# ChaoqinRobotics/LINS---LiDAR-inertial-SLAM

Hardware: NVIDIA H100
Metric: ESKF iterations/sec (higher is better)
Workload: dtype f64 (f32 association)

## Files before the change

lins---lidar-inertial-slam_b200/csrc/cuda/lins_assoc.cuh:

```cuda
#pragma once
#include "lins_assoc_az.cuh"

namespace lins_dev {

#ifndef LINS_SEARCH_DIAG
#define LINS_SEARCH_DIAG 0
#endif
constexpr bool kSearchDiag = LINS_SEARCH_DIAG != 0;
#ifndef LINS_GROUP_LANES
#define LINS_GROUP_LANES 4
#endif
constexpr int kGroupLanes = LINS_GROUP_LANES;
#ifndef LINS_THREAD_SCAN_BINS
#define LINS_THREAD_SCAN_BINS 16
#endif
#ifndef LINS_THREAD_WALK_BINS
#define LINS_THREAD_WALK_BINS 48
#endif
constexpr int kThreadScanBins = LINS_THREAD_SCAN_BINS, kThreadWalkBins = LINS_THREAD_WALK_BINS;

struct PassBuffers {
  float4* qpt;
  float4* sel;
  unsigned long long* key;
  int* pos;
  float4* qa;
  int4* qw;
  float4* qref;
  float4* qref2;
  int* qccr;
  float4* qext;
  int* wl;
  double* wacc;
  int* wcnt;
  int nvw;
};

struct PassLayout {
  size_t slots;
  size_t fixed_bytes;
  size_t query_bytes;
};

__host__ __device__ constexpr size_t align16(size_t b) { return (b + 15) & ~(size_t)15; }

__host__ __device__ __forceinline__ PassLayout pass_layout(int nslots, int qtile, PassBuffers* pb = nullptr, unsigned char* smem = nullptr,
                                                           unsigned char* qscratch = nullptr, unsigned cta = 0, size_t qscratch_stride = 0) {
  static_assert(sizeof(Smem) % 16 == 0, "slots are indexed as an array");
  const int NQ = nslots * qtile;
  const size_t nvw_all = (size_t)nslots * (qtile / 32);
  const size_t wacc_bytes = align16(nvw_all * kNAcc * sizeof(double)), wcnt_bytes = align16(nvw_all * 2 * sizeof(int));
  PassLayout lay;
  lay.slots = align16(sizeof(CtaMem));
  lay.fixed_bytes = lay.slots + nslots * sizeof(Smem) + wacc_bytes + wcnt_bytes;
  lay.query_bytes = align16((size_t)NQ * (sizeof(*pb->qpt) + sizeof(*pb->sel) + sizeof(*pb->qa) + sizeof(*pb->qw) + sizeof(*pb->qref) +
                                          sizeof(*pb->qref2) + sizeof(*pb->qext) + sizeof(*pb->key) + 3 * sizeof(*pb->pos) +
                                          sizeof(*pb->qccr) + sizeof(*pb->wl)));
  if (pb) {
    PassBuffers& b = *pb;
    b.nvw = qtile / 32;
    unsigned char* p = smem + lay.slots;
    p += nslots * sizeof(Smem);
    b.wacc = reinterpret_cast<double*>(p); p += wacc_bytes;
    b.wcnt = reinterpret_cast<int*>(p); p += wcnt_bytes;
    if (qscratch) p = qscratch + (size_t)cta * qscratch_stride;
    b.qpt = reinterpret_cast<float4*>(p); p = reinterpret_cast<unsigned char*>(b.qpt + NQ);
    b.sel = reinterpret_cast<float4*>(p); p = reinterpret_cast<unsigned char*>(b.sel + NQ);
    b.qa = reinterpret_cast<float4*>(p); p = reinterpret_cast<unsigned char*>(b.qa + NQ);
    b.qw = reinterpret_cast<int4*>(p); p = reinterpret_cast<unsigned char*>(b.qw + NQ);
    b.qref = reinterpret_cast<float4*>(p); p = reinterpret_cast<unsigned char*>(b.qref + NQ);
    b.qref2 = reinterpret_cast<float4*>(p); p = reinterpret_cast<unsigned char*>(b.qref2 + NQ);
    b.qext = reinterpret_cast<float4*>(p); p = reinterpret_cast<unsigned char*>(b.qext + NQ);
    b.key = reinterpret_cast<unsigned long long*>(p); p = reinterpret_cast<unsigned char*>(b.key + NQ);
    b.pos = reinterpret_cast<int*>(p); p = reinterpret_cast<unsigned char*>(b.pos + 3 * NQ);
    b.qccr = reinterpret_cast<int*>(p); p = reinterpret_cast<unsigned char*>(b.qccr + NQ);
    b.wl = reinterpret_cast<int*>(p);
  }
  return lay;
}

__device__ __forceinline__ AzIndex az_index_of(const Smem& sm, const BatchView& bv, bool surf) {
  AzIndex ix;
  if (surf) { ix.pts = bv.az_s + sm.ts0; ix.bstart = sm.azTabS; ix.elev = sm.elevS; ix.nb = sm.nbS; ix.nrings = sm.nringsS; ix.T = sm.Ts; }
  else { ix.pts = bv.az_c + sm.tc0; ix.bstart = sm.azTabC; ix.elev = sm.elevC; ix.nb = sm.nbC; ix.nrings = sm.nringsC; ix.T = sm.Tc; }
  return ix;
}

__device__ __forceinline__ int slot_of(int v, int Q) { return (v >= Q) + (v >= 2 * Q) + (v >= 3 * Q); }

template <int MODE>
__device__ void association_pass(CtaMem& cta, Smem* slots, const BatchView& bv, const KParams& kp, const PassBuffers& pb) {
  const int Q = bv.qtile, NQ = bv.nslots * Q;
  const float nearf = (float)kp.nearest_sq;
  const int warp = threadIdx.x >> 5, lane = threadIdx.x & 31;
  const int toff = cta.pass_first ? 32 : 0;

  for (int v = threadIdx.x; v < NQ; v += kThreads) {
    const int sl = slot_of(v, Q), i = v - sl * Q;
    Smem& sm = slots[sl];
    if (!sm.run || i >= sm.ns + sm.nc) continue;
    const float4 s = transform_to_start(pb.qpt[v], sm, kp.scan_period);
    pb.sel[v] = s;
    pb.key[v] = kKeyMax;
    const bool search = (sm.iter % kp.icp_freq) == 0;
    if (!search) {
      if (!sm.pos_valid) {
        if (i < sm.ns) { const int* o = bv.ind_s + 3 * (size_t)(sm.qs0 + i); pb.pos[3 * v] = o[0]; pb.pos[3 * v + 1] = o[1]; pb.pos[3 * v + 2] = o[2]; }
        else { const int* o = bv.ind_c + 2 * (size_t)(sm.qc0 + i - sm.ns); pb.pos[3 * v] = o[0]; pb.pos[3 * v + 1] = o[1]; pb.pos[3 * v + 2] = -1; }
      }
      continue;
    }
    if (!sm.az_ok) continue;
    const bool surf = i < sm.ns;
    const bool seeded = !sm.first_pass;
    const AzIndex ixq = az_index_of(sm, bv, surf);
    float4 qa = make_float4(0.f, 0.f, -1.f, 0.f);
    if (seeded) {
      const float4 r1 = pb.qref[v], r2 = pb.qref2[v], ex = pb.qext[v];
      const unsigned nearbits = __float_as_uint(nearf);
      const int w1s = pb.pos[3 * v], w2s = pb.pos[3 * v + 1], w3s = pb.pos[3 * v + 2];
      const int r1s = __float_as_int(ex.y), r2s = __float_as_int(ex.z), r3s = __float_as_int(ex.w);
      const int ccr0 = pb.qccr[v];
      const bool walks = ccr0 >= 0;
      auto entry = [&](int slot, bool use) -> float4 {
        return use && slot >= 0 && slot < ixq.T ? ixq.pts[slot] : make_float4(0.f, 0.f, 0.f, 0.f);
      };
      const float4 tw1 = entry(w1s, true), tr1 = entry(r1s, w1s >= 0);
      const float4 tw2 = entry(w2s, walks), tr2 = entry(r2s, walks && w2s >= 0);
      const float4 tw3 = entry(w3s, walks && surf), tr3 = entry(r3s, walks && surf && w3s >= 0);
      const float moved1 = sqrtf(sqdist_f32(s.x, s.y, s.z, r1.x, r1.y, r1.z));
      const bool ok1 = w1s >= 0 ? cert_accepted<false>(tw1, tr1, s, r1s, r1.w, moved1, nearbits, 0) : cert_rejected(r1.w, moved1);
      bool ok2 = false;
      if (ok1 && walks) {
        const int c0 = ccr0 & 0x00ffffff;
        const float moved2 = sqrtf(sqdist_f32(s.x, s.y, s.z, r2.x, r2.y, r2.z));
        ok2 = w2s >= 0 ? cert_accepted<true>(tw2, tr2, s, r2s, r2.w, moved2, nearbits, c0) : cert_rejected(r2.w, moved2);
        if (ok2 && surf) ok2 = w3s >= 0 ? cert_accepted<true>(tw3, tr3, s, r3s, ex.x, moved2, nearbits, c0) : cert_rejected(ex.x, moved2);
      }
      if (ok1 && (ok2 || ccr0 < 0)) { pb.qw[v] = make_int4(-2, 0, 0, 0); continue; }
      if (ok1) { az_polar(s, qa); pb.qa[v] = qa; pb.qw[v] = make_int4(-3, 0, 0, 0); continue; }
    }
    const int w1 = az_prepare_nn(ixq, s, nearf, seeded ? pb.pos[3 * v] : -1, (int)pb.qpt[v].w, qa);
    pb.qa[v] = qa;
    pb.qw[v] = make_int4(w1, 0, 0, 0);
    if (sm.first_pass && w1 >= 0 && (w1 & 0xffff) <= kThreadScanBins) pb.wl[NQ - 1 - atomicAdd(&cta.wl_tn[0], 1)] = v;
    else pb.wl[atomicAdd(&cta.wl_n[0], 1)] = v;
    if (bv.timers && w1 >= 0) atomicAdd(&cta.dbg[0], w1 & 0xffff);
  }
  __syncthreads();
  LINS_TICK(3 + toff);

  if (cta.any_indexed) {
    if (bv.timers && threadIdx.x == 0) {
      atomicAdd((unsigned long long*)&bv.timers[10], (unsigned long long)cta.wl_n[0]);
      atomicAdd((unsigned long long*)&bv.timers[12], (unsigned long long)cta.dbg[0]);
    }
    const float gate = sqrtf(nearf);
    auto nn_finish = [&](int v, const AzIndex& ix, const float4 s, const Top3& top, int w1, float Bout) {
      const unsigned long long k1 = top.k1;
      const int p1 = top.p1;
      const float d1 = __uint_as_float((unsigned)(k1 >> 32));
      const bool acc1 = k1 != kKeyMax && p1 >= 0 && (double)d1 < kp.nearest_sq;
      const float bound1 = w1 < 0 ? -1.f : acc1 ? cert_bound(top.d3, Bout) : rejected_slack((unsigned)(k1 >> 32), Bout, gate);
      pb.qref[v] = make_float4(s.x, s.y, s.z, bound1);
      pb.qext[v].y = __int_as_float(acc1 ? top.p2 : -1);
      pb.pos[3 * v] = acc1 ? p1 : -1;
      pb.qccr[v] = acc1 ? ((slot_ring(ix.pts[p1].w) << 24) | (int)(unsigned)(k1 & 0xffffffffu)) : -1;
    };
    constexpr int G = kGroupLanes;
    const int sub = lane & (G - 1), glead = lane & ~(G - 1);
    const unsigned gmask = G == 32 ? 0xffffffffu : (((1u << G) - 1u) << glead);
    for (;;) {
      int k = 0;
      if (sub == 0) k = atomicAdd(&cta.wl_thead[0], 1);
      k = __shfl_sync(gmask, k, glead);
      if (k >= cta.wl_tn[0]) break;
      const int v = pb.wl[NQ - 1 - k];
      const int sl = slot_of(v, Q), i = v - sl * Q;
      const Smem& sm = slots[sl];
      const AzIndex ix = az_index_of(sm, bv, i < sm.ns);
      const float4 s = pb.sel[v];
      const int w1 = pb.qw[v].x;
      const float4 qag = pb.qa[v];
      const Top3 top = az_scan_nn_group<G>(ix, s, w1, qag.y, qag.w, sub, gmask);
      if (sub == 0) nn_finish(v, ix, s, top, w1, qag.w);
    }
    for (;;) {
      int k = 0;
      if (lane == 0) k = atomicAdd(&cta.wl_head[0], 1);
      k = __shfl_sync(0xffffffffu, k, 0);
      if (k >= cta.wl_n[0]) break;
      const int v = pb.wl[k];
      const int sl = slot_of(v, Q), i = v - sl * Q;
      const Smem& sm = slots[sl];
      int w1 = pb.qw[v].x;
      Top3 top;
      top.init();
      const bool surf = i < sm.ns;
      const AzIndex ix = az_index_of(sm, bv, surf);
      const float4 s = pb.sel[v];
      float4 qa = pb.qa[v];
      if (w1 >= 0) {
        const int wp = sm.first_pass ? az_probe_window(ix, qa, w1) : -1;
        if (wp >= 0) {
          const Top3 pr = az_scan_nn(ix, s, wp, qa.y, sqrtf(widen(kProbeSq)));
          if (pr.p1 >= 0) {
            w1 = az_nn_window(ix, az_seed_bound(ix, s, pr.p1, nearf), qa);
            if (lane == 0) pb.qa[v] = qa;
          }
        }
        top = az_scan_nn(ix, s, w1, qa.y, qa.w);
      }
      if (lane == 0) nn_finish(v, ix, s, top, w1, qa.w);
    }
    __syncthreads();
    LINS_TICK(4 + toff);
    for (int v = threadIdx.x; v < NQ; v += kThreads) {
      const int sl = slot_of(v, Q), i = v - sl * Q;
      const Smem& sm = slots[sl];
      if (!sm.run || !sm.az_ok || i >= sm.ns + sm.nc || (sm.iter % kp.icp_freq) != 0) continue;
      const int lvl = pb.qw[v].x;
      if (lvl == -2) continue;
      const bool surf = i < sm.ns;
      const int ccr = pb.qccr[v];
      if (ccr < 0) {
        pb.pos[3 * v + 1] = -1; pb.pos[3 * v + 2] = -1;
        pb.qw[v] = make_int4(-1, 0, 0, 0);
        if (surf) { int* o = bv.ind_s + 3 * (size_t)(sm.qs0 + i); o[0] = -1; o[1] = -1; o[2] = -1; }
        else { int* o = bv.ind_c + 2 * (size_t)(sm.qc0 + i - sm.ns); o[0] = -1; o[1] = -1; }
        continue;
      }
      int w2 = 0, w3 = 0;
      float B2 = 0.f, B3 = 0.f;
      const bool seeded = !sm.first_pass;
      const int sd2 = seeded ? pb.pos[3 * v + 1] : -1, sd3 = seeded ? pb.pos[3 * v + 2] : -1;
      const int c = ccr & 0x00ffffff, cr = (int)((unsigned)ccr >> 24);
      const AzIndex ix = az_index_of(sm, bv, surf);
      const int p1 = pb.pos[3 * v];
      if (surf) az_prepare_walk<true>(ix, pb.sel[v], pb.qa[v], p1, c, cr, sd2, sd3, min(sm.ns, sm.Ts), nearf, w2, w3, B2, B3);
      else az_prepare_walk<false>(ix, pb.sel[v], pb.qa[v], p1, c, cr, sd2, sd3, min(sm.nc, sm.Tc), nearf, w2, w3, B2, B3);
      pb.qw[v] = make_int4(1, w2, w3, ccr);
      reinterpret_cast<float2*>(pb.key)[v] = make_float2(B2, B3);
      if (sm.first_pass && (w2 & 0xffff) <= kThreadWalkBins && (w3 & 0xffff) <= kThreadWalkBins) pb.wl[NQ - 1 - atomicAdd(&cta.wl_tn[1], 1)] = v;
      else pb.wl[atomicAdd(&cta.wl_n[1], 1)] = v;
      if (bv.timers) atomicAdd(&cta.dbg[1], (w2 & 0xffff) + 4 * (w3 & 0xffff));
    }
    __syncthreads();
    if (bv.timers && threadIdx.x == 0) {
      atomicAdd((unsigned long long*)&bv.timers[11], (unsigned long long)cta.wl_n[1]);
      atomicAdd((unsigned long long*)&bv.timers[13], (unsigned long long)cta.dbg[1]);
    }
    auto walk_finish = [&](int v, const Smem& sm, int i, bool surf, const float4 s, int ccr, const WalkOut& wo) {
      pb.pos[3 * v + 1] = wo.pos2; pb.pos[3 * v + 2] = wo.pos3;
      pb.qref2[v] = make_float4(s.x, s.y, s.z, wo.bound2);
      float4 ex = pb.qext[v];
      ex.x = wo.bound3; ex.z = __int_as_float(wo.run2); ex.w = __int_as_float(wo.run3);
      pb.qext[v] = ex;
      const int i1 = ccr & 0x00ffffff;
      if (surf) { int* o = bv.ind_s + 3 * (size_t)(sm.qs0 + i); o[0] = i1; o[1] = wo.i2; o[2] = wo.i3; }
      else { int* o = bv.ind_c + 2 * (size_t)(sm.qc0 + i - sm.ns); o[0] = i1; o[1] = wo.i2; }
    };
    for (;;) {
      int k = 0;
      if (sub == 0) k = atomicAdd(&cta.wl_thead[1], 1);
      k = __shfl_sync(gmask, k, glead);
      if (k >= cta.wl_tn[1]) break;
      const int v = pb.wl[NQ - 1 - k];
      const int sl = slot_of(v, Q), i = v - sl * Q;
      const Smem& sm = slots[sl];
      const int4 w = pb.qw[v];
      const bool surf = i < sm.ns;
      const float2 B = reinterpret_cast<const float2*>(pb.key)[v];
      const float4 s = pb.sel[v];
      const AzIndex ix = az_index_of(sm, bv, surf);
      const WalkOut wo = surf ? az_scan_walk_group<true, G>(ix, s, w.w, w.y, w.z, min(sm.ns, sm.Ts), nearf, B.x, B.y, sub, gmask)
                              : az_scan_walk_group<false, G>(ix, s, w.w, w.y, w.z, min(sm.nc, sm.Tc), nearf, B.x, B.y, sub, gmask);
      if (sub == 0) walk_finish(v, sm, i, surf, s, w.w, wo);
    }
    for (;;) {
      int k = 0;
      if (lane == 0) k = atomicAdd(&cta.wl_head[1], 1);
      k = __shfl_sync(0xffffffffu, k, 0);
      if (k >= cta.wl_n[1]) break;
      const int v = pb.wl[k];
      const int sl = slot_of(v, Q), i = v - sl * Q;
      const Smem& sm = slots[sl];
      const int4 w = pb.qw[v];
      const bool surf = i < sm.ns;
      const float2 B = reinterpret_cast<const float2*>(pb.key)[v];
      const int w2 = w.y, w3 = w.z;
      const float4 s = pb.sel[v];
      const AzIndex ix = az_index_of(sm, bv, surf);
      const WalkOut wo = surf ? az_scan_walk<true>(ix, s, w.w, w2, w3, min(sm.ns, sm.Ts), nearf, B.x, B.y)
                              : az_scan_walk<false>(ix, s, w.w, w2, w3, min(sm.nc, sm.Tc), nearf, B.x, B.y);
      if (lane == 0) walk_finish(v, sm, i, surf, s, w.w, wo);
    }
  }
  if (cta.any_legacy) {
    for (int sl = 0; sl < bv.nslots; ++sl) {
      const Smem& sm = slots[sl];
      if (!sm.run || sm.az_ok || (sm.iter % kp.icp_freq) != 0) continue;
      const bool sep = nn_separate(bv, sm.scan);
      const float4* __restrict__ nnS = sep ? bv.nn_s + bv.nn_s_off[sm.scan] : bv.ts + sm.ts0;
      const float4* __restrict__ nnC = sep ? bv.nn_c + bv.nn_c_off[sm.scan] : bv.tc + sm.tc0;
      const int TnS = sep ? bv.nn_s_off[sm.scan + 1] - bv.nn_s_off[sm.scan] : sm.Ts;
      const int TnC = sep ? bv.nn_c_off[sm.scan + 1] - bv.nn_c_off[sm.scan] : sm.Tc;
      if (sm.ns > 0 && TnS > 0) nn_brute(pb.sel + sl * Q, pb.key + sl * Q, sm.ns, nnS, TnS);
      if (sm.nc > 0 && TnC > 0) nn_brute(pb.sel + sl * Q + sm.ns, pb.key + sl * Q + sm.ns, sm.nc, nnC, TnC);
    }
    __syncthreads();
    for (int sl = 0; sl < bv.nslots; ++sl) {
      const Smem& sm = slots[sl];
      if (!sm.run || sm.az_ok || (sm.iter % kp.icp_freq) != 0) continue;
      const float4* __restrict__ tgtS = bv.ts + sm.ts0;
      const float4* __restrict__ tgtC = bv.tc + sm.tc0;
      const int fwdS = min(sm.ns, sm.Ts), fwdC = min(sm.nc, sm.Tc);
      for (int i = threadIdx.x; i < sm.ns + sm.nc; i += kThreads) {
        const int v = sl * Q + i;
        const bool surf = i < sm.ns;
        const unsigned long long k1 = pb.key[v];
        const float d1 = __uint_as_float((unsigned)(k1 >> 32));
        const int c = (int)(unsigned)(k1 & 0xffffffffu);
        const bool found = (k1 != kKeyMax) && ((double)d1 < kp.nearest_sq) && c < (surf ? sm.Ts : sm.Tc);
        int i1 = -1, i2 = -1, i3 = -1;
        if (found) {
          i1 = c;
          const float4 s = pb.sel[v];
          if (surf) walk_seq<true>(s, c, tgtS, sm.Ts, fwdS, nearf, i2, i3);
          else walk_seq<false>(s, c, tgtC, sm.Tc, fwdC, nearf, i2, i3);
        }
        pb.pos[3 * v] = i1; pb.pos[3 * v + 1] = i2; pb.pos[3 * v + 2] = i3;
        if (surf) { int* o = bv.ind_s + 3 * (size_t)(sm.qs0 + i); o[0] = i1; o[1] = i2; o[2] = i3; }
        else { int* o = bv.ind_c + 2 * (size_t)(sm.qc0 + i - sm.ns); o[0] = i1; o[1] = i2; }
      }
    }
  }
  __syncthreads();
  LINS_TICK(5 + toff);
  if (threadIdx.x == kThreads - 1) { cta.wl_n[0] = 0; cta.wl_n[1] = 0; cta.wl_tn[0] = 0; cta.wl_tn[1] = 0; cta.wl_head[0] = 0; cta.wl_head[1] = 0; cta.wl_thead[0] = 0; cta.wl_thead[1] = 0; cta.dbg[0] = 0; cta.dbg[1] = 0; }

  double* const fold_stage = cta.u.fold[warp];
  for (int v0 = warp * 32; v0 < NQ; v0 += kThreads) {
    const int sl = slot_of(v0, Q), i0 = v0 - sl * Q;
    const Smem& sm = slots[sl];
    const int ntot = sm.ns + sm.nc;
    if (!sm.run || i0 >= ntot) continue;
    const int v = v0 + lane, i = i0 + lane;
    const bool valid = i < ntot;
    const bool surf = i < sm.ns;
    const bool search = (sm.iter % kp.icp_freq) == 0;
    const bool weighted = sm.iter >= kp.icp_freq;
    const bool by_slot = search ? (sm.az_ok != 0) : (sm.pos_valid && sm.pos_is_slot);
    float4 coeff = make_float4(0.f, 0.f, 0.f, 0.f);
    float4 s = make_float4(0.f, 0.f, 0.f, 0.f);
    bool ok = false;
    if (valid) {
      const int i1 = pb.pos[3 * v], i2 = pb.pos[3 * v + 1], i3 = pb.pos[3 * v + 2];
      s = pb.sel[v];
      if (surf) {
        if (i2 >= 0 && i3 >= 0 && i1 >= 0 && i1 < sm.Ts && i2 < sm.Ts && i3 < sm.Ts) {
          const float4* t = by_slot ? bv.az_s + sm.ts0 : bv.ts + sm.ts0;
          ok = plane_residual(s, t[i1], t[i2], t[i3], weighted, coeff);
        }
      } else {
        if (i2 >= 0 && i1 >= 0 && i1 < sm.Tc && i2 < sm.Tc) {
          const float4* t = by_slot ? bv.az_c + sm.tc0 : bv.tc + sm.tc0;
          ok = line_residual(s, t[i1], t[i2], weighted, coeff);
        }
      }
    }
    double g[6] = {0.0, 0.0, 0.0, 0.0, 0.0, 0.0}, r = 0.0;
    if (ok) {
      if (MODE == MODE_ICP_REDUCE) jacobian_row_icp(pb.qpt[v], coeff, sm.phi, kp.scan_period, g, r);
      else jacobian_row(pb.qpt[v], coeff, sm.R, kp.lidar_scale, g, r);
    }
    const int vw = sl * pb.nvw + (i0 >> 5);
    warp_fold_mma(g, r, fold_stage, pb.wacc + vw * kNAcc);
    const unsigned mS = __ballot_sync(0xffffffffu, ok && surf), mC = __ballot_sync(0xffffffffu, ok && !surf);
    if (lane == kNAcc) pb.wcnt[vw * 2] = __popc(mS);
    else if (lane == kNAcc + 1) pb.wcnt[vw * 2 + 1] = __popc(mC);
    if (MODE == MODE_ASSOC && valid) {
      if (surf) {
        const size_t o = (size_t)(sm.qs0 + i);
        if (bv.sel_s) { bv.sel_s[3 * o] = s.x; bv.sel_s[3 * o + 1] = s.y; bv.sel_s[3 * o + 2] = s.z; }
        if (bv.coeff_s) { bv.coeff_s[4 * o] = coeff.x; bv.coeff_s[4 * o + 1] = coeff.y; bv.coeff_s[4 * o + 2] = coeff.z; bv.coeff_s[4 * o + 3] = coeff.w; }
        if (bv.mask_s) bv.mask_s[o] = ok ? 1 : 0;
      } else {
        const size_t o = (size_t)(sm.qc0 + i - sm.ns);
        if (bv.sel_c) { bv.sel_c[3 * o] = s.x; bv.sel_c[3 * o + 1] = s.y; bv.sel_c[3 * o + 2] = s.z; }
        if (bv.coeff_c) { bv.coeff_c[4 * o] = coeff.x; bv.coeff_c[4 * o + 1] = coeff.y; bv.coeff_c[4 * o + 2] = coeff.z; bv.coeff_c[4 * o + 3] = coeff.w; }
        if (bv.mask_c) bv.mask_c[o] = ok ? 1 : 0;
      }
    }
  }
  __syncthreads();
  LINS_TICK(6 + toff);
}

}
```

lins---lidar-inertial-slam_b200/csrc/cuda/lins_assoc_az.cuh:

```cuda
#pragma once
#include "lins_kernels.cuh"

namespace lins_dev {

struct AzIndex {
  const float4* pts;
  const aztab_t* bstart;
  const int (*elev)[2];
  int nb, nrings, T;
};
__device__ __forceinline__ int float_key(float f) { const int i = __float_as_int(f); return i >= 0 ? i : i ^ 0x7fffffff; }
__device__ __forceinline__ float key_float(int k) { return __int_as_float(k >= 0 ? k : k ^ 0x7fffffff); }
__device__ __forceinline__ float slope_of(float x, float y, float z) {
  return __fdiv_rn(z, sqrtf(__fadd_rn(__fmul_rn(x, x), __fmul_rn(y, y))));
}
__device__ __forceinline__ float ring_lower_bound(const AzIndex& ix, int r, float zq, float rq) {
  const float lo = key_float(ix.elev[r][0]), hi = key_float(ix.elev[r][1]);
  const float a = __fmaf_rn(lo, rq, -zq), b = __fmaf_rn(-hi, rq, zq);
  const float m = a > b ? lo : hi;
  const float bound = fmaxf(a, b) * rsqrtf(__fmaf_rn(m, m, 1.f)) * 0.998f - 1.0e-4f;
  return hi - lo < 1.0e30f ? bound : -1.f;
}

__device__ __forceinline__ int az_bin(float x, float y, int nb) {
// ... 307 lines not shown
  }
  {
    const int bq = az_bin_of_angle(qa.x, ix.nb);
    float& U = SURF ? U3 : U2;
    float4 t[8];
    bool ok[8];
#pragma unroll
    for (int k = 0; k < 4; ++k) {
      const int r = cr + (k < 2 ? k - 2 : k - 1);
      const bool rok = r >= 0 && r < ix.nrings;
      const int slot = rok ? (int)ix.bstart[r * ix.nb + bq] : -1;
      t[2 * k] = fetch(slot, ok[2 * k]);
      t[2 * k + 1] = fetch(rok ? slot - 1 : -1, ok[2 * k + 1]);
    }
#pragma unroll
    for (int k = 0; k < 8; ++k) U = seed_bound<SURF, !SURF>(t[k], ok[k], s, c, cr, fwdBound, U);
  }
  int blo, nbins;
  const float Uw2 = widen(U2);
  az_window(ix.nb, qa.x, az_halfwidth(Uw2, qa.y), blo, nbins);
  w2 = pack_window(blo, nbins);
  B2 = nbins >= ix.nb ? 3.0e38f : sqrtf(Uw2);
  if (SURF) {
    const float Uw3 = widen(U3);
    az_window(ix.nb, qa.x, az_halfwidth(Uw3, qa.y), blo, nbins);
    w3 = pack_window(blo, nbins);
    B3 = nbins >= ix.nb ? 3.0e38f : sqrtf(Uw3);
  } else { w3 = w2; B3 = B2; }
}

#ifndef LINS_WALK_IN_FLIGHT
#define LINS_WALK_IN_FLIGHT 4
#endif
constexpr int kWalkInFlight = LINS_WALK_IN_FLIGHT;
#ifndef LINS_GROUP_WALK_IN_FLIGHT
#define LINS_GROUP_WALK_IN_FLIGHT 4
#endif
constexpr int kGroupWalkInFlight = LINS_GROUP_WALK_IN_FLIGHT;
struct WalkOut {
  int i2, i3, pos2, pos3, run2, run3;
  float bound2, bound3;
};
template <bool SURF>
__device__ __forceinline__ WalkOut az_scan_walk(const AzIndex& ix, const float4 s, int ccr, int w2, int w3, int fwdBound, float nearf,
                                                float B2, float B3) {
  const int lane = threadIdx.x & 31;
  const int c = ccr & 0x00ffffff, cr = (int)((unsigned)ccr >> 24);
  Top3 top;
  top.init();
  constexpr int LPR = SURF ? 7 : 8;
  const int q = lane / LPR;
  const bool own = SURF && q >= 4;
  const int r = own ? cr : cr + (q < 2 ? q - 2 : q - 1);
  const int sub = own ? lane - 4 * LPR : lane - q * LPR, step = own ? 4 : LPR;
  const bool cls2 = SURF ? own : true;
  if (r >= 0 && r < ix.nrings) {
    const int win = cls2 ? w2 : w3;
    const int blo = win >> 16, nbins = win & 0xffff, base = r * ix.nb;
    for (int seg = 0; seg < 2; ++seg) {
      int p, pe;
      if (seg == 0) { p = ix.bstart[base + blo]; pe = ix.bstart[base + min(blo + nbins, ix.nb)]; }
      else { const int e1 = blo + nbins - ix.nb; if (e1 <= 0) break; p = ix.bstart[base]; pe = ix.bstart[base + e1]; }
      for (p += sub; p < pe; p += kWalkInFlight * step) {
        float4 tt[kWalkInFlight];
#pragma unroll
        for (int u = 0; u < kWalkInFlight; ++u) tt[u] = ld_slot(ix, p + step * u < pe ? p + step * u : p);
#pragma unroll
        for (int u = 0; u < kWalkInFlight; ++u) {
          const int pu = p + step * u;
          const float4 t = tt[u];
          const unsigned d = __float_as_uint(sqdist_f32(t.x, t.y, t.z, s.x, s.y, s.z));
          const int j = slot_index(t.w);
          const bool fwd = j > c;
          const bool adm = pu < pe && j != c && (!fwd || j < fwdBound);
          const unsigned long long k = adm ? (((unsigned long long)d << 32) | (fwd ? order_fwd(j) : order_bwd(j))) : kKeyMax;
          top.insert(k, pu);
        }
      }
    }
  }
  const float gate = sqrtf(nearf);
  const unsigned nearbits = __float_as_uint(nearf);
  const bool mine2 = cls2;
  Top3 neutral;
  neutral.init();
  WalkOut o;
  auto finish = [&](Top3 t, float Bout, int& idx, int& pos, int& run, float& bound) {
    warp_top3(t);
    const bool ok = (unsigned)(t.k1 >> 32) < nearbits && t.p1 >= 0;
    idx = ok ? order_decode((unsigned)(t.k1 & 0xffffffffu)) : -1;
    pos = ok ? t.p1 : -1;
    run = ok ? t.p2 : -1;
    bound = ok ? cert_bound(t.d3, Bout) : rejected_slack((unsigned)(t.k1 >> 32), Bout, gate);
  };
  finish(mine2 ? top : neutral, B2, o.i2, o.pos2, o.run2, o.bound2);
  if (SURF) finish(mine2 ? neutral : top, B3, o.i3, o.pos3, o.run3, o.bound3);
  else { o.i3 = -1; o.pos3 = -1; o.run3 = -1; o.bound3 = 0.f; }
  return o;
}

template <bool SURF, int G>
__device__ __forceinline__ WalkOut az_scan_walk_group(const AzIndex& ix, const float4 s, int ccr, int w2, int w3, int fwdBound, float nearf,
                                                      float B2, float B3, int sub, unsigned gmask) {
  const int c = ccr & 0x00ffffff, cr = (int)((unsigned)ccr >> 24);
  Top3 t2, t3;
  t2.init(); t3.init();
  auto scan_ring = [&](int r, int win, Top3& top, int start, int step) {
    const int blo = win >> 16, nbins = win & 0xffff, base = r * ix.nb;
    for (int seg = 0; seg < 2; ++seg) {
      int p, pe;
      if (seg == 0) { p = ix.bstart[base + blo]; pe = ix.bstart[base + min(blo + nbins, ix.nb)]; }
      else { const int e1 = blo + nbins - ix.nb; if (e1 <= 0) break; p = ix.bstart[base]; pe = ix.bstart[base + e1]; }
      for (p += start; p < pe; p += kGroupWalkInFlight * step) {
        float4 tt[kGroupWalkInFlight];
#pragma unroll
        for (int u = 0; u < kGroupWalkInFlight; ++u) tt[u] = ld_slot(ix, p + u * step < pe ? p + u * step : p);
#pragma unroll
        for (int u = 0; u < kGroupWalkInFlight; ++u) {
          const int pu = p + u * step;
          const float4 t = tt[u];
          const unsigned d = __float_as_uint(sqdist_f32(t.x, t.y, t.z, s.x, s.y, s.z));
          const int j = slot_index(t.w);
          const bool fwd = j > c;
          const bool adm = pu < pe && j != c && (!fwd || j < fwdBound);
          top.insert(adm ? (((unsigned long long)d << 32) | (fwd ? order_fwd(j) : order_bwd(j))) : kKeyMax, pu);
        }
      }
    }
  };
  if (SURF && cr < ix.nrings) scan_ring(cr, w2, t2, sub, G);
  for (int idx = sub; idx < 4; idx += G) {
    const int r = cr + (idx < 2 ? idx - 2 : idx - 1);
    if (r < 0 || r >= ix.nrings) continue;
    if (SURF) scan_ring(r, w3, t3, 0, 1); else scan_ring(r, w2, t2, 0, 1);
  }
  group_top3<G>(t2, gmask);
  if (SURF) group_top3<G>(t3, gmask);
  const float gate = sqrtf(nearf);
  const unsigned nearbits = __float_as_uint(nearf);
  WalkOut o;
  auto finish = [&](const Top3& t, float Bout, int& idx, int& pos, int& run, float& bound) {
    const bool ok = (unsigned)(t.k1 >> 32) < nearbits && t.p1 >= 0;
    idx = ok ? order_decode((unsigned)(t.k1 & 0xffffffffu)) : -1;
    pos = ok ? t.p1 : -1;
    run = ok ? t.p2 : -1;
    bound = ok ? cert_bound(t.d3, Bout) : rejected_slack((unsigned)(t.k1 >> 32), Bout, gate);
  };
  finish(t2, B2, o.i2, o.pos2, o.run2, o.bound2);
  if (SURF) finish(t3, B3, o.i3, o.pos3, o.run3, o.bound3);
  else { o.i3 = -1; o.pos3 = -1; o.run3 = -1; o.bound3 = 0.f; }
  return o;
}

template <bool WALK>
__device__ __forceinline__ bool cert_accepted(const float4 tw, const float4 tr, const float4 s, int r, float bound, float moved, unsigned nearbits,
                                              int c) {
  auto key_of = [&](const float4 t) -> unsigned long long {
    const unsigned d = __float_as_uint(sqdist_f32(t.x, t.y, t.z, s.x, s.y, s.z));
    const int j = slot_index(t.w);
    const unsigned lo = WALK ? (j > c ? order_fwd(j) : order_bwd(j)) : (unsigned)j;
    return ((unsigned long long)d << 32) | lo;
  };
  const unsigned long long kw = key_of(tw);
  const unsigned dw = (unsigned)(kw >> 32);
  if (!(dw < nearbits)) return false;
  if (r >= 0 && !(kw < key_of(tr))) return false;
  return sqrtf(__uint_as_float(dw)) + moved + 2.0e-4f < bound;
}
__device__ __forceinline__ bool cert_rejected(float slack, float moved) { return slack > 0.f && 2.0f * moved + 2.0e-4f < slack; }

}
```

lins---lidar-inertial-slam_b200/csrc/cuda/lins_kernels.cuh:

```cuda
#pragma once
#include "../../../include/lins_gpu.h"
#include "lins_device_math.cuh"

namespace lins_dev {

#ifndef LINS_THREADS
#define LINS_THREADS 512
#endif
#ifndef LINS_MIN_CTAS
#define LINS_MIN_CTAS 1
#endif
constexpr int kThreads = LINS_THREADS;
constexpr int kMinCtas = LINS_MIN_CTAS;
constexpr int kWarps = kThreads / 32;
constexpr int kMaxSlots = 4;
constexpr int kMaxRing = 128;
constexpr int kNAcc = 28;
constexpr int kNNChunk = 1024;
constexpr int kAzTabS = 4096;
constexpr int kAzTabC = 1024;
constexpr float kPiF = 3.14159265358979f;
constexpr unsigned long long kKeyMax = 0xFFFFFFFFFFFFFFFFull;

enum KernelMode { MODE_IESKF = 0, MODE_ASSOC = 1, MODE_ICP_REDUCE = 2, MODE_JACOBIAN = 3 };

struct BatchView {
  int n_scans;
  const float4* qs; const int* qs_off;
  const float4* qc; const int* qc_off;
  const float4* ts; const int* ts_off;
  const float4* tc; const int* tc_off;
  const float4* nn_s; const int* nn_s_off;
  const float4* nn_c; const int* nn_c_off;
  const unsigned char* nn_stale;
  const double* state_in;
  const double* cov_in;
  double* state_out;
  double* cov_out;
  lins_scan_result* results;
  lins_report* reports;
  int* ind_s;
  int* ind_c;
  float* sel_s; float* sel_c;
  float* coeff_s; float* coeff_c;
  unsigned char* mask_s; unsigned char* mask_c;
  double* accum;
  float4* az_s; float4* az_c;
  int* work_counter;
  long long* timers;
  int qtile;
  int nslots;
  const int* icp_done;
  unsigned char* qscratch;
  size_t qscratch_stride;
};

struct IcpState {
  double matP[36];
  int iters, converged, done, pad;
};
constexpr int kIcpDoneStride = (int)(sizeof(IcpState) / sizeof(int));
static_assert(sizeof(IcpState) % sizeof(int) == 0, "IcpState stride");

struct KParams {
  int num_iter, icp_freq, force_all_iters, mode, iter0;
  double nearest_sq, lidar_std, lidar_scale, scan_period;
};

__device__ __forceinline__ bool nn_separate(const BatchView& bv, int scan) {
  return bv.nn_s != nullptr && (bv.nn_stale == nullptr || bv.nn_stale[scan] != 0);
}

__device__ __forceinline__ unsigned long long pack_key(float d, unsigned int lo) {
  return ((unsigned long long)__float_as_uint(d) << 32) | lo;
}
__device__ __forceinline__ unsigned long long shfl_xor_u64(unsigned long long v, int m) {
  return __shfl_xor_sync(0xffffffffu, v, m);
}
__device__ __forceinline__ unsigned long long warp_min_u64(unsigned long long v) {
#pragma unroll
  for (int m = 16; m > 0; m >>= 1) {
    unsigned long long o = shfl_xor_u64(v, m);
    v = o < v ? o : v;
  }
  return v;
}

typedef unsigned short aztab_t;

struct alignas(16) Smem {
  double prior[20];
  double Pc[18 * 6];
  double lin[20];
  double phi[3];
  double R[9];
  double Rinv[9];
  double dvec[18];
  double acc[kNAcc + 4];
  double A6[36];
  double y6[6];
  double M6[36];
  double X6[6];
  double upd[18];
  double residualNorm;
  int flags[4];
  int cnt[2];
  int scan;
  int iter;
  int fresh;
  int run;
  int finished;
  int first_pass;
  int pos_valid, pos_is_slot;
  int qs0, ns, qc0, nc, ts0, Ts, tc0, Tc;
  int sortedS, sortedC;
  int az_ok;
  int nbS, nbC, nringsS, nringsC;
  aztab_t azTabS[kAzTabS + 2];
  aztab_t azTabC[kAzTabC + 2];
  int elevS[kMaxRing][2], elevC[kMaxRing][2];
};

struct CtaMem {
  union {
    unsigned build_tab[kAzTabS / 2 + 1];
    struct { double P[324], X[324], U[108], V[108], X6[72]; } ex;
    double fold[kWarps][64];
  } u;
  int scan_tmp[kThreads];
  int wl_n[2], wl_head[2];
  int wl_tn[2], wl_thead[2];
  int dbg[2];
  int n_active, any_fresh, any_finished, any_legacy, any_indexed, exhausted, pass_first;
  unsigned long long mbar;
  unsigned int phase;
  long long tlast;
};
static_assert(sizeof(((CtaMem*)nullptr)->u.fold) <= sizeof(((CtaMem*)nullptr)->u.build_tab), "the fold stage must not grow the CTA");

#define LINS_TICK(k)                                                                   \
  do {                                                                                 \
    if (bv.timers && threadIdx.x == 0) {                                               \
      const long long _t = clock64();                                                  \
      atomicAdd((unsigned long long*)&bv.timers[k], (unsigned long long)(_t - cta.tlast)); \
      cta.tlast = _t;                                                                   \
    }                                                                                  \
  } while (0)

__device__ __forceinline__ float4 transform_to_start(const float4 p, const Smem& sm, double scan_period) {
  float fi = p.w - (float)((int)p.w);
  double s = (1.f / scan_period) * fi;
  d3 v = mk3(s * sm.phi[0], s * sm.phi[1], s * sm.phi[2]);
  q4 r = axis2Quat(v);
  d3 P2 = mk3((double)p.x, (double)p.y, (double)p.z);
  d3 rp = qrot(r, P2);
  d3 t = mk3(s * sm.lin[0], s * sm.lin[1], s * sm.lin[2]);
  float4 o;
  o.x = (float)(rp.x + t.x); o.y = (float)(rp.y + t.y); o.z = (float)(rp.z + t.z); o.w = p.w;
  return o;
}

__device__ inline void check_ring_sorted(const float4* __restrict__ tgt, int T, int* sorted_flag) {
  if (threadIdx.x == 0) *sorted_flag = 1;
  __syncthreads();
  for (int j = threadIdx.x; j < T; j += kThreads) {
    const int rj = (int)__ldg(&tgt[j]).w;
    const int rp = j > 0 ? (int)__ldg(&tgt[j - 1]).w : -1;
    if (rj < 0 || rj >= kMaxRing || (j > 0 && rj < rp)) *sorted_flag = 0;
  }
  __syncthreads();
}

__device__ inline void nn_brute(const float4* sel, unsigned long long* key, int nq, const float4* __restrict__ tgt, int T) {
  const int warp = threadIdx.x >> 5, lane = threadIdx.x & 31;
  const int nqg = (nq + 31) >> 5, nch = (T + kNNChunk - 1) / kNNChunk;
  for (int item = warp; item < nqg * nch; item += kWarps) {
    const int qg = item % nqg, ch = item / nqg;
    const int qi = qg * 32 + lane;
    const bool valid = qi < nq;
    const float4 s = valid ? sel[qi] : make_float4(0.f, 0.f, 0.f, 0.f);
    const int j0 = ch * kNNChunk, j1 = min(T, j0 + kNNChunk);
    float best = __int_as_float(0x7f800000);
    int bi = -1;
#pragma unroll 4
    for (int j = j0; j < j1; ++j) {
      const float4 t = __ldg(&tgt[j]);
      const float d = sqdist_f32(s.x, s.y, s.z, t.x, t.y, t.z);
      if (d < best) { best = d; bi = j; }
    }
    if (valid && bi >= 0) atomicMin(&key[qi], pack_key(best, (unsigned)bi));
  }
}


__device__ __forceinline__ unsigned int order_fwd(int j) { return (unsigned)j; }
__device__ __forceinline__ unsigned int order_bwd(int j) { return 0x80000000u | (unsigned)(0x7fffffff - j); }
__device__ __forceinline__ int order_decode(unsigned int o) { return (o & 0x80000000u) ? (0x7fffffff - (int)(o & 0x7fffffffu)) : (int)o; }

template <bool SURF>
__device__ void walk_seq(const float4 s, int c, const float4* __restrict__ tgt, int T, int fwdBound, float nearf,
                         int& i2, int& i3) {
  const int cr = (int)__ldg(&tgt[c]).w;
  float m2 = nearf, m3 = nearf;
  i2 = -1; i3 = -1;
  for (int j = c + 1; j < fwdBound; ++j) {
    const float4 t = __ldg(&tgt[j]);
    const int rj = (int)t.w;
    if ((double)rj > (double)cr + 2.5) break;
    const float d = sqdist_f32(t.x, t.y, t.z, s.x, s.y, s.z);
    if (SURF) {
      if (rj <= cr) { if (d < m2) { m2 = d; i2 = j; } }
      else { if (d < m3) { m3 = d; i3 = j; } }
    } else {
      if (rj > cr) { if (d < m2) { m2 = d; i2 = j; } }
    }
  }
  for (int j = c - 1; j >= 0; --j) {
    const float4 t = __ldg(&tgt[j]);
    const int rj = (int)t.w;
    if ((double)rj < (double)cr - 2.5) break;
    const float d = sqdist_f32(t.x, t.y, t.z, s.x, s.y, s.z);
    if (SURF) {
      if (rj >= cr) { if (d < m2) { m2 = d; i2 = j; } }
      else { if (d < m3) { m3 = d; i3 = j; } }
    } else {
      if (rj < cr) { if (d < m2) { m2 = d; i2 = j; } }
    }
  }
}

__device__ __forceinline__ bool plane_residual(const float4 sel, const float4 t1, const float4 t2, const float4 t3,
                                               bool weighted, float4& coeff) {
  d3 P0 = mk3(sel.x, sel.y, sel.z), P1 = mk3(t1.x, t1.y, t1.z), P2 = mk3(t2.x, t2.y, t2.z), P3 = mk3(t3.x, t3.y, t3.z);
  d3 M = cross3(sub3(P1, P2), sub3(P1, P3));
  double r = dot3(sub3(P0, P1), M);
  double m = norm3(M);
  float res = (float)(r / m);
  d3 jac = div3(M, m);
  float s = 1.f;
  if (weighted) {
    float n2 = __fadd_rn(__fadd_rn(__fmul_rn(sel.x, sel.x), __fmul_rn(sel.y, sel.y)), __fmul_rn(sel.z, sel.z));
    float rt = sqrtf(sqrtf(n2));
    s = (float)(1.0 - 1.8 * (double)fabsf(res) / (double)rt);
  }
  if ((double)s > 0.1 && res != 0.f) {
    coeff.x = (float)((double)s * jac.x); coeff.y = (float)((double)s * jac.y); coeff.z = (float)((double)s * jac.z);
    coeff.w = __fmul_rn(s, res);
    return true;
  }
  return false;
}
__device__ __forceinline__ bool line_residual(const float4 sel, const float4 t1, const float4 t2, bool weighted,
                                              float4& coeff) {
  d3 P0 = mk3(sel.x, sel.y, sel.z), P1 = mk3(t1.x, t1.y, t1.z), P2 = mk3(t2.x, t2.y, t2.z);
  d3 P = cross3(sub3(P0, P1), sub3(P0, P2));
  float r = (float)norm3(P);
  float d12 = (float)norm3(sub3(P1, P2));
  float res = __fdiv_rn(r, d12);
  d3 a = sub3(P2, P1);
  d3 num = mk3(P.y * a.z + P.z * (-a.y), P.x * (-a.z) + P.z * a.x, P.x * a.y + P.y * (-a.x));
  double den = (double)__fmul_rn(d12, r);
  d3 jac = div3(num, den);
  float s = 1.f;
  if (weighted) s = (float)(1.0 - 1.8 * (double)fabsf(res));
  if ((double)s > 0.1 && res != 0.f) {
    coeff.x = (float)((double)s * jac.x); coeff.y = (float)((double)s * jac.y); coeff.z = (float)((double)s * jac.z);
    coeff.w = __fmul_rn(s, res);
    return true;
  }
  return false;
}

__device__ __forceinline__ void jacobian_row(const float4 kp, const float4 coeff, const double* R, double lidar_scale,
                                             double* g, double& r) {
  const double cx = coeff.x, cy = coeff.y, cz = coeff.z;
  r = lidar_scale * (double)coeff.w;
  const double ux = R[0] * cx + R[3] * cy + R[6] * cz;
  const double uy = R[1] * cx + R[4] * cy + R[7] * cz;
  const double uz = R[2] * cx + R[5] * cy + R[8] * cz;
  const double px = kp.x, py = kp.y, pz = kp.z;
  g[0] = cx; g[1] = cy; g[2] = cz;
  g[3] = py * uz - pz * uy; g[4] = pz * ux - px * uz; g[5] = px * uy - py * ux;
}
__device__ __forceinline__ void jacobian_row_icp(const float4 kp, const float4 coeff, const double* phi, double scan_period,
                                                 double* g, double& b) {
  float fi = kp.w - (float)((int)kp.w);
  double s = (1.f / scan_period) * fi;
  q4 rq = axis2Quat(mk3(s * phi[0], s * phi[1], s * phi[2]));
  m3 R = qtoR(rq);
  const double cx = coeff.x, cy = coeff.y, cz = coeff.z;
  b = -0.05 * (double)coeff.w;
  const double ux = R.m[0] * cx + R.m[3] * cy + R.m[6] * cz;
  const double uy = R.m[1] * cx + R.m[4] * cy + R.m[7] * cz;
  const double uz = R.m[2] * cx + R.m[5] * cy + R.m[8] * cz;
  const double px = kp.x, py = kp.y, pz = kp.z;
  g[0] = py * uz - pz * uy; g[1] = pz * ux - px * uz; g[2] = px * uy - py * ux;
  g[3] = cx; g[4] = cy; g[5] = cz;
}

__device__ __forceinline__ double warp_fold_row(const double* g, double r) {
// ... 228 lines not shown
```

Measured before the change: 6.884 million.

## Accept certificates when runner-up overtakes winner by swapping neighbours, add cert counters

The certificate check now returns a reason code and, when the stored runner-up has become nearer than the stored winner but still satisfies the bound, it accepts by swapping winner and runner-up instead of falling back to a full search. For the nearest neighbour this skips the NN scan and goes straight to the walk stage. For the walk neighbours it rewrites the stored indices in place. Timer-gated counters that record certificate outcomes and per-pass bucketed timings are also added. These add ballots and atomics only when timers are enabled, but the swap path carries correctness risk if the runner-up is not truly the new nearest.

```diff
diff --git a/lins---lidar-inertial-slam_b200/csrc/cuda/lins_assoc.cuh b/lins---lidar-inertial-slam_b200/csrc/cuda/lins_assoc.cuh
--- a/lins---lidar-inertial-slam_b200/csrc/cuda/lins_assoc.cuh
+++ b/lins---lidar-inertial-slam_b200/csrc/cuda/lins_assoc.cuh
@@ -18,6 +18,15 @@
 #define LINS_THREAD_WALK_BINS 48
 #endif
 constexpr int kThreadScanBins = LINS_THREAD_SCAN_BINS, kThreadWalkBins = LINS_THREAD_WALK_BINS;
+
+constexpr int kCertSlots = 40, kPassSlots = 48;
+__device__ __forceinline__ void count_cert_events(long long* timers, unsigned ev) {
+#pragma unroll
+  for (int k = 0; k < 8; ++k) {
+    const unsigned n1 = __popc(__ballot_sync(0xffffffffu, (ev >> k) & 1u)), n2 = __popc(__ballot_sync(0xffffffffu, (ev >> (8 + k)) & 1u));
+    if ((threadIdx.x & 31) == 0 && (n1 | n2)) atomicAdd((unsigned long long*)&timers[kCertSlots + k], ((unsigned long long)n2 << 32) | n1);
+  }
+}
 
 struct PassBuffers {
   float4* qpt;
@@ -93,9 +102,10 @@
   const int Q = bv.qtile, NQ = bv.nslots * Q;
   const float nearf = (float)kp.nearest_sq;
   const int warp = threadIdx.x >> 5, lane = threadIdx.x & 31;
-  const int toff = cta.pass_first ? 32 : 0;
 
   for (int v = threadIdx.x; v < NQ; v += kThreads) {
+    unsigned ev = 0u;
+    do {
     const int sl = slot_of(v, Q), i = v - sl * Q;
     Smem& sm = slots[sl];
     if (!sm.run || i >= sm.ns + sm.nc) continue;
@@ -129,15 +139,26 @@
       const float4 tw2 = entry(w2s, walks), tr2 = entry(r2s, walks && w2s >= 0);
       const float4 tw3 = entry(w3s, walks && surf), tr3 = entry(r3s, walks && surf && w3s >= 0);
       const float moved1 = sqrtf(sqdist_f32(s.x, s.y, s.z, r1.x, r1.y, r1.z));
-      const bool ok1 = w1s >= 0 ? cert_accepted<false>(tw1, tr1, s, r1s, r1.w, moved1, nearbits, 0) : cert_rejected(r1.w, moved1);
+      const int c1 = w1s >= 0 ? cert_check<false>(tw1, tr1, s, r1s, r1.w, moved1, nearbits, 0)
+                              : (cert_rejected(r1.w, moved1) ? kCertKeep : kCertFailSlack);
+      const bool ok1 = c1 <= kCertSwap;
+      ev = 1u | (1u << (ok1 ? 1 : c1)) | (c1 == kCertSwap ? 1u << 7 : 0u);
+      if (c1 == kCertSwap) { az_polar(s, qa); pb.qa[v] = qa; pb.qw[v] = make_int4(-4, 0, 0, 0); continue; }
       bool ok2 = false;
+      int c2 = kCertKeep, c3 = kCertKeep;
       if (ok1 && walks) {
         const int c0 = ccr0 & 0x00ffffff;
         const float moved2 = sqrtf(sqdist_f32(s.x, s.y, s.z, r2.x, r2.y, r2.z));
-        ok2 = w2s >= 0 ? cert_accepted<true>(tw2, tr2, s, r2s, r2.w, moved2, nearbits, c0) : cert_rejected(r2.w, moved2);
-        if (ok2 && surf) ok2 = w3s >= 0 ? cert_accepted<true>(tw3, tr3, s, r3s, ex.x, moved2, nearbits, c0) : cert_rejected(ex.x, moved2);
-      }
-      if (ok1 && (ok2 || ccr0 < 0)) { pb.qw[v] = make_int4(-2, 0, 0, 0); continue; }
+        c2 = w2s >= 0 ? cert_check<true>(tw2, tr2, s, r2s, r2.w, moved2, nearbits, c0) : (cert_rejected(r2.w, moved2) ? kCertKeep : kCertFailSlack);
+        ok2 = c2 <= kCertSwap;
+        if (ok2 && surf) {
+          c3 = w3s >= 0 ? cert_check<true>(tw3, tr3, s, r3s, ex.x, moved2, nearbits, c0) : (cert_rejected(ex.x, moved2) ? kCertKeep : kCertFailSlack);
+          ok2 = c3 <= kCertSwap;
+        }
+        ev |= (1u << 8) | (1u << (8 + (ok2 ? 1 : c2 <= kCertSwap ? c3 : c2))) |
+              (ok2 && (c2 == kCertSwap || c3 == kCertSwap) ? 1u << 15 : 0u);
+      }
+      if (ok1 && (ok2 || ccr0 < 0)) { pb.qw[v] = make_int4(-2, (c2 == kCertSwap ? 1 : 0) | (c3 == kCertSwap ? 2 : 0), 0, 0); continue; }
       if (ok1) { az_polar(s, qa); pb.qa[v] = qa; pb.qw[v] = make_int4(-3, 0, 0, 0); continue; }
     }
     const int w1 = az_prepare_nn(ixq, s, nearf, seeded ? pb.pos[3 * v] : -1, (int)pb.qpt[v].w, qa);
@@ -146,9 +167,11 @@
     if (sm.first_pass && w1 >= 0 && (w1 & 0xffff) <= kThreadScanBins) pb.wl[NQ - 1 - atomicAdd(&cta.wl_tn[0], 1)] = v;
     else pb.wl[atomicAdd(&cta.wl_n[0], 1)] = v;
     if (bv.timers && w1 >= 0) atomicAdd(&cta.dbg[0], w1 & 0xffff);
+    } while (false);
+    if (bv.timers) count_cert_events(bv.timers, ev);
   }
   __syncthreads();
-  LINS_TICK(3 + toff);
+  LINS_TICK_PASS(3);
 
   if (cta.any_indexed) {
     if (bv.timers && threadIdx.x == 0) {
@@ -161,6 +184,8 @@
       const int p1 = top.p1;
       const float d1 = __uint_as_float((unsigned)(k1 >> 32));
       const bool acc1 = k1 != kKeyMax && p1 >= 0 && (double)d1 < kp.nearest_sq;
+      if (bv.timers && !slots[slot_of(v, Q)].first_pass && pb.pos[3 * v] >= 0 && acc1 && (p1 == pb.pos[3 * v] || p1 == __float_as_int(pb.qext[v].y)))
+        atomicAdd((unsigned long long*)&bv.timers[kCertSlots + 6], 1ull);
       const float bound1 = w1 < 0 ? -1.f : acc1 ? cert_bound(top.d3, Bout) : rejected_slack((unsigned)(k1 >> 32), Bout, gate);
       pb.qref[v] = make_float4(s.x, s.y, s.z, bound1);
       pb.qext[v].y = __int_as_float(acc1 ? top.p2 : -1);
@@ -214,14 +239,37 @@
       if (lane == 0) nn_finish(v, ix, s, top, w1, qa.w);
     }
     __syncthreads();
-    LINS_TICK(4 + toff);
+    if (bv.timers && threadIdx.x == 0 && !cta.pass_first) {
+      const int n = cta.wl_n[0] + cta.wl_tn[0], b = n == 0 ? 0 : n <= 16 ? 1 : 2;
+      atomicAdd((unsigned long long*)&bv.timers[kPassSlots + b], 1ull);
+      atomicAdd((unsigned long long*)&bv.timers[kPassSlots + 3 + b], (unsigned long long)(clock64() - cta.tlast));
+    }
+    LINS_TICK_PASS(4);
     for (int v = threadIdx.x; v < NQ; v += kThreads) {
       const int sl = slot_of(v, Q), i = v - sl * Q;
       const Smem& sm = slots[sl];
       if (!sm.run || !sm.az_ok || i >= sm.ns + sm.nc || (sm.iter % kp.icp_freq) != 0) continue;
-      const int lvl = pb.qw[v].x;
-      if (lvl == -2) continue;
+      const int2 lq = *reinterpret_cast<const int2*>(&pb.qw[v]);
+      const int lvl = lq.x;
       const bool surf = i < sm.ns;
+      auto swap_front = [&](int k, float* runner_up) {
+        const int w = pb.pos[3 * v + k], r = __float_as_int(*runner_up);
+        pb.pos[3 * v + k] = r;
+        *runner_up = __int_as_float(w);
+        return az_index_of(sm, bv, surf).pts[r].w;
+      };
+      if (lvl == -2) {
+        if (lq.y) {
+          int* const o = surf ? bv.ind_s + 3 * (size_t)(sm.qs0 + i) : bv.ind_c + 2 * (size_t)(sm.qc0 + i - sm.ns);
+          if (lq.y & 1) o[1] = slot_index(swap_front(1, &pb.qext[v].z));
+          if (lq.y & 2) o[2] = slot_index(swap_front(2, &pb.qext[v].w));
+        }
+        continue;
+      }
+      if (lvl == -4) {
+        const float tw = swap_front(0, &pb.qext[v].y);
+        pb.qccr[v] = (slot_ring(tw) << 24) | slot_index(tw);
+      }
       const int ccr = pb.qccr[v];
       if (ccr < 0) {
         pb.pos[3 * v + 1] = -1; pb.pos[3 * v + 2] = -1;
@@ -239,7 +287,7 @@
       const int p1 = pb.pos[3 * v];
       if (surf) az_prepare_walk<true>(ix, pb.sel[v], pb.qa[v], p1, c, cr, sd2, sd3, min(sm.ns, sm.Ts), nearf, w2, w3, B2, B3);
       else az_prepare_walk<false>(ix, pb.sel[v], pb.qa[v], p1, c, cr, sd2, sd3, min(sm.nc, sm.Tc), nearf, w2, w3, B2, B3);
-      pb.qw[v] = make_int4(1, w2, w3, ccr);
+      pb.qw[v] = make_int4(lvl == -3 ? 2 : 1, w2, w3, ccr);
       reinterpret_cast<float2*>(pb.key)[v] = make_float2(B2, B3);
       if (sm.first_pass && (w2 & 0xffff) <= kThreadWalkBins && (w3 & 0xffff) <= kThreadWalkBins) pb.wl[NQ - 1 - atomicAdd(&cta.wl_tn[1], 1)] = v;
       else pb.wl[atomicAdd(&cta.wl_n[1], 1)] = v;
@@ -251,9 +299,14 @@
       atomicAdd((unsigned long long*)&bv.timers[13], (unsigned long long)cta.dbg[1]);
     }
     auto walk_finish = [&](int v, const Smem& sm, int i, bool surf, const float4 s, int ccr, const WalkOut& wo) {
+      float4 ex = pb.qext[v];
+      if (bv.timers && pb.qw[v].x == 2) {
+        auto held = [](int w, int r, int now) { return w >= 0 ? now == w || now == r : now < 0; };
+        if (held(pb.pos[3 * v + 1], __float_as_int(ex.z), wo.pos2) && (!surf || held(pb.pos[3 * v + 2], __float_as_int(ex.w), wo.pos3)))
+          atomicAdd((unsigned long long*)&bv.timers[kCertSlots + 6], 1ull << 32);
+      }
       pb.pos[3 * v + 1] = wo.pos2; pb.pos[3 * v + 2] = wo.pos3;
       pb.qref2[v] = make_float4(s.x, s.y, s.z, wo.bound2);
-      float4 ex = pb.qext[v];
       ex.x = wo.bound3; ex.z = __int_as_float(wo.run2); ex.w = __int_as_float(wo.run3);
       pb.qext[v] = ex;
       const int i1 = ccr & 0x00ffffff;
@@ -336,7 +389,12 @@
     }
   }
   __syncthreads();
-  LINS_TICK(5 + toff);
+  if (bv.timers && threadIdx.x == 0 && !cta.pass_first) {
+    const int n = cta.wl_n[1] + cta.wl_tn[1], b = n == 0 ? 0 : n <= 16 ? 1 : n <= 32 ? 2 : 3;
+    atomicAdd((unsigned long long*)&bv.timers[kPassSlots + 6 + b], 1ull);
+    atomicAdd((unsigned long long*)&bv.timers[kPassSlots + 10 + b], (unsigned long long)(clock64() - cta.tlast));
+  }
+  LINS_TICK_PASS(5);
   if (threadIdx.x == kThreads - 1) { cta.wl_n[0] = 0; cta.wl_n[1] = 0; cta.wl_tn[0] = 0; cta.wl_tn[1] = 0; cta.wl_head[0] = 0; cta.wl_head[1] = 0; cta.wl_thead[0] = 0; cta.wl_thead[1] = 0; cta.dbg[0] = 0; cta.dbg[1] = 0; }
 
   double* const fold_stage = cta.u.fold[warp];
@@ -394,7 +452,7 @@
     }
   }
   __syncthreads();
-  LINS_TICK(6 + toff);
+  LINS_TICK_PASS(6);
 }
 
 }
diff --git a/lins---lidar-inertial-slam_b200/csrc/cuda/lins_assoc_az.cuh b/lins---lidar-inertial-slam_b200/csrc/cuda/lins_assoc_az.cuh
--- a/lins---lidar-inertial-slam_b200/csrc/cuda/lins_assoc_az.cuh
+++ b/lins---lidar-inertial-slam_b200/csrc/cuda/lins_assoc_az.cuh
@@ -483,20 +483,22 @@
   return o;
 }
 
+enum : int { kCertKeep = 0, kCertSwap = 1, kCertFailRunnerUp = 2, kCertFailBound = 3, kCertFailGate = 4, kCertFailSlack = 5 };
 template <bool WALK>
-__device__ __forceinline__ bool cert_accepted(const float4 tw, const float4 tr, const float4 s, int r, float bound, float moved, unsigned nearbits,
-                                              int c) {
+__device__ __forceinline__ int cert_check(const float4 tw, const float4 tr, const float4 s, int r, float bound, float moved, unsigned nearbits,
+                                          int c) {
   auto key_of = [&](const float4 t) -> unsigned long long {
     const unsigned d = __float_as_uint(sqdist_f32(t.x, t.y, t.z, s.x, s.y, s.z));
     const int j = slot_index(t.w);
     const unsigned lo = WALK ? (j > c ? order_fwd(j) : order_bwd(j)) : (unsigned)j;
     return ((unsigned long long)d << 32) | lo;
   };
-  const unsigned long long kw = key_of(tw);
-  const unsigned dw = (unsigned)(kw >> 32);
-  if (!(dw < nearbits)) return false;
-  if (r >= 0 && !(kw < key_of(tr))) return false;
-  return sqrtf(__uint_as_float(dw)) + moved + 2.0e-4f < bound;
+  const unsigned long long kw = key_of(tw), kr = r >= 0 ? key_of(tr) : kKeyMax;
+  const bool swap = kr < kw;
+  const unsigned dm = (unsigned)((swap ? kr : kw) >> 32);
+  if (!(dm < nearbits)) return kCertFailGate;
+  if (!(sqrtf(__uint_as_float(dm)) + moved + 2.0e-4f < bound)) return swap ? kCertFailRunnerUp : kCertFailBound;
+  return swap ? kCertSwap : kCertKeep;
 }
 __device__ __forceinline__ bool cert_rejected(float slack, float moved) { return slack > 0.f && 2.0f * moved + 2.0e-4f < slack; }
 
diff --git a/lins---lidar-inertial-slam_b200/csrc/cuda/lins_kernels.cuh b/lins---lidar-inertial-slam_b200/csrc/cuda/lins_kernels.cuh
--- a/lins---lidar-inertial-slam_b200/csrc/cuda/lins_kernels.cuh
+++ b/lins---lidar-inertial-slam_b200/csrc/cuda/lins_kernels.cuh
@@ -146,6 +146,7 @@
       cta.tlast = _t;                                                                   \
     }                                                                                  \
   } while (0)
+#define LINS_TICK_PASS(k) LINS_TICK((k) + (cta.pass_first ? 32 : 0))
 
 __device__ __forceinline__ float4 transform_to_start(const float4 p, const Smem& sm, double scan_period) {
   float fi = p.w - (float)((int)p.w);
```

New measurement: 7.263 million (median of 6 runs). 5.5% higher.
